# ielym/fastvision

Measured on AMD Instinct MI355X. Metric: images/sec (640×640, bs=32/GPU) YOLOv3 train step, 1/2/4/8 MI355X, higher is better.
Workload: dtype bf16

## Files before the change

fastvision_amd/csrc/conv_wgrad.hip:

```cpp
#include <type_traits>

#include "common.h"

namespace {

__device__ __forceinline__ void wait_vm0() { asm volatile("s_waitcnt vmcnt(0)" ::: "memory"); }
template <int N>
__device__ __forceinline__ void wait_vmcnt_n() {
    asm volatile("s_waitcnt vmcnt(%0)" ::"n"(N) : "memory");
}

__device__ __forceinline__ void slab_store(float* p, float v) { *p = v; }

struct WgradParams {
    const void* x;
    const void* dy;
    float* slab;
    int M, N, C;
    int OW, OHW;
    FastDiv div_ow, div_ohw;
    int x_img, x_row, sy, sx, x_y0, x_x0;
    int dy_img, dy_row, dy_pad, dy_pitch;
    uint32_t dy_zero_off;
    int ntaps;
// ... 298 lines not shown
    __builtin_amdgcn_sched_barrier(0);

    const int i16 = lane & 15, g = lane >> 4, q = i16 >> 2, pp = i16 & 3;
    const uint32_t lds0 = (uint32_t)(size_t)LDS_PTR(smem);
    uint32_t ra[2][4], rb[2][2];
#pragma unroll
    for (int hh = 0; hh < 2; ++hh) {
        const int row = 8 * g + 4 * hh + q;
        const int fr = (q << 2) | ((2 * g + hh) & 3);
        const int rbase = row * 256 + 8 * (pp & 1);
#pragma unroll
        for (int t = 0; t < 4; ++t) ra[hh][t] = lds0 + rbase + (((wr * 8 + t * 2 + (pp >> 1)) ^ fr) << 4);
#pragma unroll
        for (int t = 0; t < 2; ++t) rb[hh][t] = lds0 + rbase + (((wc * 4 + t * 2 + (pp >> 1)) ^ fr) << 4);
    }
    bf16x8 af[4][2], b0[2][2], b1[2][2];
    auto read_a = [&](uint32_t boff, auto kind_tag) {
        constexpr int KO = decltype(kind_tag)::value * OP;
#pragma unroll
        for (int mt = 0; mt < 4; ++mt) {
            af[mt][0] = cat8(tr_read<KO>(ra[0][mt] + boff), tr_read<KO>(ra[1][mt] + boff));
            af[mt][1] = cat8(tr_read<KO + 8192>(ra[0][mt] + boff), tr_read<KO + 8192>(ra[1][mt] + boff));
        }
    };
    auto read_b = [&](uint32_t boff, auto kind_tag, bf16x8 (&bf)[2][2]) {
        constexpr int KO = decltype(kind_tag)::value * OP;
#pragma unroll
        for (int nt = 0; nt < 2; ++nt) {
            bf[nt][0] = cat8(tr_read<KO>(rb[0][nt] + boff), tr_read<KO>(rb[1][nt] + boff));
            bf[nt][1] = cat8(tr_read<KO + 8192>(rb[0][nt] + boff), tr_read<KO + 8192>(rb[1][nt] + boff));
        }
    };
    auto mma = [&](int ha, int hb, bf16x8 (&bf)[2][2]) {
        __builtin_amdgcn_s_setprio(1);
#pragma unroll
        for (int kk = 0; kk < 2; ++kk)
#pragma unroll
            for (int mt = 0; mt < 4; ++mt)
#pragma unroll
                for (int nt = 0; nt < 2; ++nt)
                    acc[ha * 4 + mt][hb * 2 + nt] =
                        __builtin_amdgcn_mfma_f32_16x16x32_bf16(af[mt][kk], bf[nt][kk], acc[ha * 4 + mt][hb * 2 + nt], 0, 0, 0);
        __builtin_amdgcn_s_setprio(0);
    };
    auto retire_reads_then_barrier = [&]() {
        asm volatile("s_waitcnt lgkmcnt(0)" ::: "memory");
        __builtin_amdgcn_s_barrier();
        __builtin_amdgcn_sched_barrier(0);
    };
    using K0 = std::integral_constant<int, 0>;
    using K1 = std::integral_constant<int, 1>;
    using K2 = std::integral_constant<int, 2>;
    using K3 = std::integral_constant<int, 3>;

    uint32_t d1[2], x1[2], d2[2], x2[2];
    {
        uint32_t d0[2], x0[2];
        decode(0, d0, x0);
        stage(2, 0, d0, x0); stage(0, 0, d0, x0); stage(3, 0, d0, x0); stage(1, 0, d0, x0);
    }
    decode(1, d1, x1);
    decode(2, d2, x2);
    if (steps > 1) {
        stage(2, 1, d1, x1); stage(0, 1, d1, x1); stage(3, 1, d1, x1);
        wait_vmcnt_n<6>();
    } else {
        wait_vmcnt_n<0>();
    }
    __builtin_amdgcn_s_barrier();
    stamp(1);
    if (wr == 1) __builtin_amdgcn_s_barrier();

    for (int s = 0; s < steps; ++s) {
        const int cur = s & 1;
        const uint32_t boff = (uint32_t)cur * BUF;
        read_b(boff, K2{}, b0);
        read_a(boff, K0{});
        if (s + 1 < steps) stage(1, cur ^ 1, d1, x1);
        retire_reads_then_barrier();
        mma(0, 0, b0);
        __builtin_amdgcn_s_barrier();
        read_b(boff, K3{}, b1);
        if (s + 2 < steps) stage(2, cur, d2, x2);
        retire_reads_then_barrier();
        mma(0, 1, b1);
        __builtin_amdgcn_s_barrier();
        read_a(boff, K1{});
        if (s + 2 < steps) stage(0, cur, d2, x2);
        retire_reads_then_barrier();
        mma(1, 1, b1);
        __builtin_amdgcn_s_barrier();
        if (s + 2 < steps) {
            stage(3, cur, d2, x2);
            wait_vmcnt_n<6>();
        } else {
            wait_vmcnt_n<0>();
        }
        d1[0] = d2[0]; d1[1] = d2[1]; x1[0] = x2[0]; x1[1] = x2[1];
        decode(s + 3, d2, x2);
        __builtin_amdgcn_s_barrier();
        __builtin_amdgcn_sched_barrier(0);
        mma(1, 0, b0);
        __builtin_amdgcn_s_barrier();
    }
    if (wr == 0) __builtin_amdgcn_s_barrier();
    stamp(2);

    float* out = p.slab + (int64_t)ks * p.ntaps * p.N * p.C;
    const int r = lane & 15;
#pragma unroll
    for (int mi = 0; mi < 8; ++mi)
#pragma unroll
        for (int ni = 0; ni < 4; ++ni) {
            const int j = wc * 64 + ni * 16 + r;
            int tap, c;
            if (p.tpt > 1) {
                const int ts = j / p.C;
                tap = tg * p.tpt + ts;
                c = j - ts * p.C;
            } else {
                tap = tg;
                c = c0 + j;
            }
            if (c < p.C && tap < p.ntaps) {
#pragma unroll
                for (int jj = 0; jj < 4; ++jj) {
                    const int n = n0 + wr * 128 + mi * 16 + g * 4 + jj;
                    if (n < p.N) slab_store(out + ((int64_t)tap * p.N + n) * p.C + c, acc[mi][ni][jj]);
                }
            }
        }
    stamp(3);
}

struct PwgradParams {
    const void* x;
    const void* dy;
    float* slab;
    int B, OH, OW;
    int x_img, x_row, x_y0, x_x0;
    int dy_img, dy_row, dy_pad;
    int tx, ty, tiles, per_block;
    int runs;
    FastDiv div_tx, div_img;
};

template <int V>
struct IntC {
    static constexpr int value = V;
};
template <int I, int N, class F>
__device__ __forceinline__ void static_for(F&& f) {
    if constexpr (I < N) {
        f(IntC<I>{});
        static_for<I + 1, N>(f);
    }
}

template <int C, int NTOT, int STRIDE, int TH>
__global__ __launch_bounds__(256, (C == 32 && TH * STRIDE <= 4) ? 3 : 2) void pwgrad_kernel(const PwgradParams p) {
    constexpr int TW = 32, NB = 64, NH = NTOT / NB;
    constexpr int XW = STRIDE * TW + 2, XH = STRIDE * (TH - 1) + 3, XPIX = XW * XH;
    constexpr int XROWB = C * 2, YROWB = NB * 2;
    constexpr int XPPI = 1024 / XROWB, YPPI = 1024 / YROWB;
    constexpr int X_INSTR = (XPIX + XPPI - 1) / XPPI, Y_INSTR = TH * TW / YPPI;
    constexpr int X_BYTES = X_INSTR * 1024;
    constexpr int WC = C / 16, WN = 4 / WC;
    constexpr int NT = NB / 16 / WN, CT = 9;
    static_assert(9 * (C / 16) == WC * CT && WN * WC == 4, "nine column tiles per wave");
    static_assert((TH - 1) * STRIDE * XW * XROWB + 4 * XROWB < 65536 && (TH - 1) * 32 * YROWB + 4 * YROWB < 65536, "ds_read immediates");
    extern __shared__ __attribute__((aligned(16))) char smem[];
    char* const xs = smem;
    char* const ys = smem + X_BYTES;
    const int tid = threadIdx.x, lane = tid & 63, w = tid >> 6;
    const int wn = w / WC, wc = w % WC;
    const int i16 = lane & 15, g = lane >> 4, q = i16 >> 2, pp = i16 & 3;

    int run, nh;
    if (NH == 1) {
        run = blockIdx.x;
        nh = 0;
    } else {
        const int t = blockIdx.x >> 3;
        nh = t & 1;
        run = (t >> 1) * 8 + (blockIdx.x & 7);
        if (run >= p.runs) return;
    }

    auto xswz = [](int lcol) { return C == 32 ? (lcol >> 3) & 1 : ((lcol >> 1) & 1) | (((lcol >> 3) & 1) << 1); };
    auto yswz = [](int row) { return ((row >> 1) & 1) | (((row >> 3) & 1) << 1); };
    const uint32_t lds_x = (uint32_t)(size_t)LDS_PTR(xs), lds_y = (uint32_t)(size_t)LDS_PTR(ys);

    uint32_t ya[NT], xa[CT][2];
#pragma unroll
    for (int nt = 0; nt < NT; ++nt) {
        const int row0 = 8 * g + q;
        ya[nt] = lds_y + row0 * YROWB + (((wn * NT + nt) ^ yswz(row0)) << 5) + pp * 8;
    }
#pragma unroll
    for (int ct = 0; ct < CT; ++ct) {
        const int gct = wc * CT + ct;
        const int tap = gct / (C / 16), blk = gct % (C / 16);
        const int tyy = tap / 3, txx = tap - 3 * tyy;
        const int off = STRIDE == 1 ? txx : (txx & 1) * (XW / 2) + (txx >> 1);
#pragma unroll
        for (int h = 0; h < 2; ++h) {
            const int lcol = off + 8 * g + q + 4 * h;
            xa[ct][h] = lds_x + (tyy * XW + lcol) * XROWB + ((blk ^ xswz(lcol)) << 5) + pp * 8;
        }
    }

    f32x4 acc[NT][CT];
#pragma unroll
    for (int i = 0; i < NT; ++i)
#pragma unroll
        for (int j = 0; j < CT; ++j) acc[i][j] = f32x4{0.f, 0.f, 0.f, 0.f};

    const int t_begin = run * p.per_block;
    const int t_end = t_begin + p.per_block < p.tiles ? t_begin + p.per_block : p.tiles;
    const int Hx = p.x_img / p.x_row;
#pragma unroll 1
    for (int tile = t_begin; tile < t_end; ++tile) {
        const int b = (int)fd_div((uint32_t)tile, p.div_img);
        const int trem = tile - b * (p.tx * p.ty);
        const int tyi = (int)fd_div((uint32_t)trem, p.div_tx), txi = trem - tyi * p.tx;
        const int oy0 = tyi * TH, ox0 = txi * TW;
        __syncthreads();
        {
        {
            const bf16_t* src0 = (const bf16_t*)p.x + (int64_t)b * p.x_img * C;
#pragma unroll 1
            for (int i = 0; i < (X_INSTR + 3) / 4; ++i) {
                const int j = i * 4 + w;
                if (j < X_INSTR) {
                    const int row = j * XPPI + lane / (XROWB / 16);
                    const int pix = row < XPIX ? row : XPIX - 1;
                    const int py = STRIDE == 1 ? (pix * 1928) >> 16 : (pix * 993) >> 16;
                    const int lcol = pix - py * XW;
                    const int px = STRIDE == 1 ? lcol : (lcol < XW / 2 ? 2 * lcol : 2 * (lcol - XW / 2) + 1);
                    int iy = STRIDE * oy0 + p.x_y0 + py, ix = STRIDE * ox0 + p.x_x0 + px;
                    iy = iy < Hx ? iy : Hx - 1;
                    ix = ix < p.x_row ? ix : p.x_row - 1;
                    const int chunk = (lane % (XROWB / 16)) ^ (xswz(lcol) << 1);
                    __builtin_amdgcn_global_load_lds(GLB_PTR(src0 + ((int64_t)iy * p.x_row + ix) * C + chunk * 8), LDS_PTR(xs + j * 1024), 16, 0, 0);
                }
            }
        }
        {
            const bf16_t* src0 = (const bf16_t*)p.dy + (int64_t)b * p.dy_img * NTOT + nh * NB;
#pragma unroll 1
            for (int i = 0; i < (Y_INSTR + 3) / 4; ++i) {
                const int j = i * 4 + w;
                if (j < Y_INSTR) {
                    const int row = j * YPPI + lane / (YROWB / 16);
                    const int oy = oy0 + (row >> 5), ox = ox0 + (row & 31);
                    const bool in = oy < p.OH && ox < p.OW;
                    const int64_t pix = in ? (int64_t)(oy + p.dy_pad) * p.dy_row + ox + p.dy_pad : 0;
                    const int chunk = (lane % (YROWB / 16)) ^ (yswz(row) << 1);
                    __builtin_amdgcn_global_load_lds(GLB_PTR(src0 + pix * NTOT + chunk * 8), LDS_PTR(ys + j * 1024), 16, 0, 0);
                }
            }
        }
        }
        wait_vm0();
        __syncthreads();
        static_for<0, TH>([&](auto rc) {
            constexpr int r = decltype(rc)::value;
            constexpr int XO = r * STRIDE * XW * XROWB, YO = r * 32 * YROWB;
            constexpr int CG = C == 32 ? 9 : 5;
            bf16x8 af[NT];
#pragma unroll
            for (int nt = 0; nt < NT; ++nt) af[nt] = cat8(tr_read<YO>(ya[nt]), tr_read<YO + 4 * YROWB>(ya[nt]));
#pragma unroll
            for (int c0 = 0; c0 < CT; c0 += CG) {
                bf16x8 bfr[CG];
#pragma unroll
                for (int ct = c0; ct < (c0 + CG < CT ? c0 + CG : CT); ++ct) bfr[ct - c0] = cat8(tr_read<XO>(xa[ct][0]), tr_read<XO>(xa[ct][1]));
                asm volatile("s_waitcnt lgkmcnt(0)" ::: "memory");
                __builtin_amdgcn_sched_barrier(0);
#pragma unroll
                for (int nt = 0; nt < NT; ++nt)
#pragma unroll
                    for (int ct = c0; ct < (c0 + CG < CT ? c0 + CG : CT); ++ct)
                        acc[nt][ct] = __builtin_amdgcn_mfma_f32_16x16x32_bf16(af[nt], bfr[ct - c0], acc[nt][ct], 0, 0, 0);
                __builtin_amdgcn_sched_barrier(0);
            }
        });
    }
    float* out = p.slab + (int64_t)run * 9 * NTOT * C;
#pragma unroll
    for (int nt = 0; nt < NT; ++nt)
#pragma unroll
        for (int ct = 0; ct < CT; ++ct) {
            const int gct = wc * CT + ct;
            const int tap = gct / (C / 16), c = (gct % (C / 16)) * 16 + i16;
#pragma unroll
            for (int j = 0; j < 4; ++j) {
                const int n = nh * NB + (wn * NT + nt) * 16 + g * 4 + j;
                slab_store(out + ((int64_t)tap * NTOT + n) * C + c, acc[nt][ct][j]);
            }
        }
}

__global__ __launch_bounds__(256) void wgrad_reduce_kernel(const float* __restrict__ slab, float* __restrict__ dw, int N, int C,
                                                           int ntaps, int ksplit, int accumulate) {
    __shared__ float part[4][9][64];
    __shared__ float outs[64 * 9];
    const int64_t nc = (int64_t)N * C;
    const int64_t i0 = (int64_t)blockIdx.x * 64;
    const int li = threadIdx.x & 63, grp = threadIdx.x >> 6;
    const int64_t i = i0 + li;
    for (int t = 0; t < ntaps; ++t) {
        float s = 0.f;
        if (i < nc) {
            const float* src = slab + (int64_t)t * nc + i;
            int k = grp;
            for (; k + 12 < ksplit; k += 16) {
                const float v0 = src[(int64_t)k * ntaps * nc], v1 = src[(int64_t)(k + 4) * ntaps * nc];
                const float v2 = src[(int64_t)(k + 8) * ntaps * nc], v3 = src[(int64_t)(k + 12) * ntaps * nc];
                s += (v0 + v1) + (v2 + v3);
            }
            for (; k < ksplit; k += 4) s += src[(int64_t)k * ntaps * nc];
        }
        part[grp][t][li] = s;
    }
    __syncthreads();
    for (int e = threadIdx.x; e < 64 * ntaps; e += 256) {
        const int t = e / 64, l = e - t * 64;
        outs[l * ntaps + t] = (part[0][t][l] + part[1][t][l]) + (part[2][t][l] + part[3][t][l]);
    }
    __syncthreads();
    const int64_t valid = (nc - i0 < 64 ? nc - i0 : 64) * ntaps;
    for (int e = threadIdx.x; e < valid; e += 256) {
        float* o = dw + i0 * ntaps + e;
        *o = accumulate ? *o + outs[e] : outs[e];
    }
}

template <int TAPS>
__global__ __launch_bounds__(1024) void wgrad_reduce4_kernel(const float* __restrict__ slab, float* __restrict__ dw, int N, int C,
                                                             int ksplit, int accumulate, int kg) {
    extern __shared__ float rsm[];
    float* part = rsm;
    float* outs = rsm + kg * TAPS * 256;
    const int64_t nc = (int64_t)N * C;
    const int64_t i0 = (int64_t)blockIdx.x * 256;
    const int li = threadIdx.x & 63, grp = threadIdx.x >> 6;
    const int64_t i = i0 + li * 4;
    const int64_t kstride = (int64_t)TAPS * nc;
    f32x4 s[TAPS];
#pragma unroll
    for (int t = 0; t < TAPS; ++t) s[t] = f32x4{0.f, 0.f, 0.f, 0.f};
    if (i < nc) {
        const float* src = slab + i;
        constexpr int KU = TAPS == 1 ? 8 : 4;
        int k = grp;
        for (; k + (KU - 1) * kg < ksplit; k += KU * kg) {
            f32x4 v[KU][TAPS];
#pragma unroll
            for (int u = 0; u < KU; ++u)
#pragma unroll
                for (int t = 0; t < TAPS; ++t) v[u][t] = *(const f32x4*)(src + (int64_t)(k + u * kg) * kstride + (int64_t)t * nc);
#pragma unroll
            for (int u = 0; u < KU; ++u)
#pragma unroll
                for (int t = 0; t < TAPS; ++t) s[t] += v[u][t];
        }
        for (; k < ksplit; k += kg) {
            f32x4 v[TAPS];
#pragma unroll
            for (int t = 0; t < TAPS; ++t) v[t] = *(const f32x4*)(src + (int64_t)k * kstride + (int64_t)t * nc);
#pragma unroll
            for (int t = 0; t < TAPS; ++t) s[t] += v[t];
        }
    }
#pragma unroll
    for (int t = 0; t < TAPS; ++t) *(f32x4*)(part + ((grp * TAPS + t) * 256 + li * 4)) = s[t];
    __syncthreads();
    for (int e = threadIdx.x; e < 256 * TAPS; e += blockDim.x) {
        const int t = e / 256, l = e - t * 256;
        float a = 0.f;
        for (int g = 0; g < kg; ++g) a += part[(g * TAPS + t) * 256 + l];
        outs[l * TAPS + t] = a;
    }
    __syncthreads();
    const int64_t valid = (nc - i0 < 256 ? nc - i0 : 256) * TAPS;
    for (int e = threadIdx.x; e < valid; e += blockDim.x) {
        float* o = dw + i0 * TAPS + e;
        *o = accumulate ? *o + outs[e] : outs[e];
    }
}

__global__ __launch_bounds__(1024) void wgrad_reduce_tap_kernel(const float* __restrict__ slab, float* __restrict__ dw, int64_t nc, int ksplit,
                                                                int accumulate) {
    __shared__ f32x4 part[16][64];
    const int t = blockIdx.y;
    const int64_t i0 = (int64_t)blockIdx.x * 256;
    const int li = threadIdx.x & 63, w = threadIdx.x >> 6;
    const int64_t i = i0 + li * 4;
    const int64_t kstride = 9 * nc;
    f32x4 s = f32x4{0.f, 0.f, 0.f, 0.f};
    if (i < nc) {
        const float* src = slab + (int64_t)t * nc + i;
        int k = w;
        for (; k + 7 * 16 < ksplit; k += 8 * 16) {
            f32x4 v[8];
#pragma unroll
            for (int u = 0; u < 8; ++u) v[u] = *(const f32x4*)(src + (int64_t)(k + u * 16) * kstride);
#pragma unroll
            for (int u = 0; u < 8; ++u) s += v[u];
        }
        for (; k < ksplit; k += 16) s += *(const f32x4*)(src + (int64_t)k * kstride);
    }
    part[w][li] = s;
    __syncthreads();
    if (threadIdx.x < 256) {
        const int l = threadIdx.x;
        float a = 0.f;
#pragma unroll
        for (int g = 0; g < 16; ++g) a += part[g][l >> 2][l & 3];
        if (i0 + l < nc) {
            float* o = dw + (i0 + l) * 9 + t;
            *o = accumulate ? *o + a : a;
        }
    }
}

struct WgradPlan {
    int tile, ntn, ntc, ntaps, ksplit, mchunk, M, OH, OW, tpt, ngroups;
};

inline bool wgrad_thin_enabled() {
    static bool v = [] {
        const char* e = getenv("FVA_WGRAD_THIN");
        return !e || atoi(e) != 0;
    }();
    return v;
}
inline bool wgrad8_enabled() {
    static bool v = [] {
        const char* e = getenv("FVA_WGRAD8");
        return !e || atoi(e) != 0;
    }();
    return v;
}
inline bool use_wgrad8(const fva_conv_desc* d) {
    if (!wgrad8_enabled() || d->dtype != FVA_BF16 || d->ksize != 3 || d->Cout % 256 || !(d->Cin == 128 || d->Cin % 256 == 0)) return false;
    const int64_t OH = (d->H - 1) / d->stride + 1, OW = (d->W - 1) / d->stride + 1, M = d->B * OH * OW;
    const int64_t units = (int64_t)(d->Cout / 256) * cdiv(d->Cin, 256) * (d->Cin == 128 ? 5 : 9);
    return M * units >= 24ll * 64 * 256;
}

int g_wgrad_plan_beside = 0;
int plan_wgrad(const fva_conv_desc* d, WgradPlan& pl, bool beside = false) {
    pl.tile = d->dtype == FVA_BF16 ? (use_wgrad8(d) ? 256 : 128) : 64;
    pl.OH = (d->H - 1) / d->stride + 1;
    pl.OW = (d->W - 1) / d->stride + 1;
    pl.M = d->B * pl.OH * pl.OW;
    pl.ntn = cdiv(d->Cout, pl.tile);
    pl.ntc = cdiv(d->Cin, pl.tile);
    pl.ntaps = d->ksize * d->ksize;
    pl.tpt = (d->Cin < pl.tile && pl.tile % d->Cin == 0 && pl.ntaps > 1) ? pl.tile / d->Cin : 1;
    pl.ngroups = cdiv(pl.ntaps, pl.tpt);
    const int tiles = pl.ntn * pl.ntc * pl.ngroups;
    const int max_by_m = cdiv(pl.M, 256) > 0 ? cdiv(pl.M, 256) : 1;
    const int64_t per = (int64_t)pl.ntaps * d->Cout * d->Cin * 4;
    int64_t max_by_ws = (512ll << 20) / per;
    int kmax = max_by_m < 1024 ? max_by_m : 1024;
    if (kmax > max_by_ws) kmax = (int)max_by_ws;
    if (kmax < 1) kmax = 1;
    static const int slots8 = [] { const char* e = getenv("FVA_WGRAD_SLOTS8"); return e && atoi(e) > 0 ? atoi(e) : 0; }();
    static const int slots4 = [] { const char* e = getenv("FVA_WGRAD_SLOTS"); return e && atoi(e) > 0 ? atoi(e) : 0; }();
    const int slots = pl.tile == 256 ? (slots8 ? slots8 : beside ? 128 : 256) : (slots4 ? slots4 : beside ? 256 : 512);
    const double t_full = 2.0 * pl.M * pl.tile * pl.tile / (pl.tile == 256 ? 4.3e12 : 1.6e12);
    const double t_slab = (double)per * 2.0 / 3.0e12 + 0.05e-6;
    int ks = 1;
    double best = 1e30;
    for (int k = 1; k <= kmax; ++k) {
        const int rounds = cdiv((int64_t)tiles * k, slots);
        const double cost = rounds * t_full / k + k * t_slab;
        if (cost < best * (1.0 - 1e-9)) { best = cost; ks = k; }
    }
    pl.mchunk = cdiv(cdiv(pl.M, ks), 64) * 64;
    pl.ksplit = cdiv(pl.M, pl.mchunk);
    return FVA_OK;
}

inline bool use_pwgrad(const fva_conv_desc* d) {
    static const bool on = [] { const char* e = getenv("FVA_PWGRAD"); return !e || atoi(e) != 0; }();
    if (!on || d->dtype != FVA_BF16 || d->ksize != 3 || !((d->Cin == 32 && d->Cout == 64) || (d->Cin == 64 && d->Cout == 128))) return false;
    const int OW = (d->W - 1) / d->stride + 1, OH = (d->H - 1) / d->stride + 1;
    return OW >= 32 && OH >= 8 && d->in_pad >= 1 && d->dy_pad >= 1;
}
struct PwgradPlan {
    int th, tx, ty, tiles, runs, per_block, grid;
};
inline int pwgrad_th(const fva_conv_desc* d) {
    static int th1 = 0, th2 = 0;
    static const bool init = [] {
        const char* e = getenv("FVA_PWGRAD_TH");
        if (e) {
            int a = 0, b = 0;
            const int n = sscanf(e, "%d,%d", &a, &b);
            if (n >= 1 && (a == 8 || a == 4)) th1 = a;
            if (n >= 2 && (b == 4 || b == 2)) th2 = b;
        }
        return true;
    }();
    (void)init;
    if (d->stride == 1) return th1 ? th1 : 8;
    return th2 ? th2 : (d->Cin == 64 ? 2 : 4);
}
inline void plan_pwgrad(const fva_conv_desc* d, PwgradPlan& pl, bool beside) {
    const int OH = (d->H - 1) / d->stride + 1, OW = (d->W - 1) / d->stride + 1;
    pl.th = pwgrad_th(d);
    pl.tx = cdiv(OW, 32);
    pl.ty = cdiv(OH, pl.th);
    pl.tiles = d->B * pl.tx * pl.ty;
    const int nh = d->Cout / 64;
    static const int per_cu = [] { const char* e = getenv("FVA_PWGRAD_SLOTS"); return e ? atoi(e) : 2; }();
    int slots = 256 * per_cu / nh;
    if (beside) slots /= 2;
    const int runs = pl.tiles < slots ? pl.tiles : slots;
    pl.per_block = cdiv(pl.tiles, runs);
    pl.runs = cdiv(pl.tiles, pl.per_block);
    pl.grid = nh == 1 ? pl.runs : cdiv(pl.runs, 8) * 16;
}

template <int C, int N, int STRIDE, int TH>
int launch_pwgrad(const PwgradParams& p, int grid, hipStream_t s) {
    constexpr int XPIX = (STRIDE * 32 + 2) * (STRIDE * (TH - 1) + 3);
    constexpr int XPPI = 1024 / (C * 2);
    constexpr int smem = ((XPIX + XPPI - 1) / XPPI) * 1024 + (TH * 32 / 8) * 1024;
    static bool attr_done = false;
    if (!attr_done) {
        (void)hipFuncSetAttribute((const void*)pwgrad_kernel<C, N, STRIDE, TH>, hipFuncAttributeMaxDynamicSharedMemorySize, smem);
        attr_done = true;
    }
    hipLaunchKernelGGL((pwgrad_kernel<C, N, STRIDE, TH>), dim3(grid), dim3(256), smem, s, p);
    FVA_LAUNCH_CHECK("pwgrad_kernel");
    fva_note_kernel("pwgrad");
    return FVA_OK;
}
template <int C, int N>
int launch_pwgrad_any(const PwgradParams& p, int stride, int th, int grid, hipStream_t s) {
    if (stride == 1) return th == 8 ? launch_pwgrad<C, N, 1, 8>(p, grid, s) : launch_pwgrad<C, N, 1, 4>(p, grid, s);
    return th == 4 ? launch_pwgrad<C, N, 2, 4>(p, grid, s) : launch_pwgrad<C, N, 2, 2>(p, grid, s);
}

}

extern "C" {

int64_t fva_conv_wgrad_workspace(const fva_conv_desc* d) {
    if (!d) return 0;
    WgradPlan pl, pb;
    plan_wgrad(d, pl, false);
    plan_wgrad(d, pb, true);
    int ks = pl.ksplit > pb.ksplit ? pl.ksplit : pb.ksplit;
    if (use_pwgrad(d)) {
        PwgradPlan pp;
        plan_pwgrad(d, pp, false);
        ks = ks > pp.runs ? ks : pp.runs;
    }
    return (int64_t)ks * pl.ntaps * d->Cout * d->Cin * 4;
}

int fva_conv_wgrad_plan(int beside) {
    const int prev = g_wgrad_plan_beside;
    if (beside == 0 || beside == 1) g_wgrad_plan_beside = beside;
    return prev;
}

int fva_conv_wgrad(const fva_conv_desc* d, const void* x, const void* dy, float* dw, int accumulate, void* workspace,
                   int64_t workspace_bytes, void* stream) {
    if (!d || !x || !dy || !dw || !workspace) return fva_fail(FVA_ERR_ARG, "fva_conv_wgrad: null pointer");
    if (d->dtype != FVA_F32 && d->dtype != FVA_BF16) return fva_fail(FVA_ERR_ARG, "fva_conv_wgrad: bad dtype");
    if (!((d->ksize == 1 && d->stride == 1) || (d->ksize == 3 && (d->stride == 1 || d->stride == 2))))
        return fva_fail(FVA_ERR_ARG, "fva_conv_wgrad: unsupported ksize/stride");
    const int epc = d->dtype == FVA_BF16 ? 8 : 4;
    if (d->Cin % epc || d->Cout % epc) return fva_fail(FVA_ERR_ARG, "fva_conv_wgrad: channels must be multiples of %d", epc);
    if (d->in_pad < d->ksize / 2) return fva_fail(FVA_ERR_ARG, "fva_conv_wgrad: in_pad too small");
    if (d->dy_pad < 1) return fva_fail(FVA_ERR_ARG, "fva_conv_wgrad: dy buffer needs a zero border (dy_pad >= 1)");
    const int64_t esz = d->dtype == FVA_BF16 ? 2 : 4;
    if ((int64_t)d->B * (d->H + 2 * d->in_pad) * (d->W + 2 * d->in_pad) * d->Cin * esz >= (1ll << 32) ||
        (int64_t)d->B * (d->H + 2) * (d->W + 2) * d->Cout * esz >= (1ll << 32))
        return fva_fail(FVA_ERR_ARG, "fva_conv_wgrad: operand larger than 4 GiB (32-bit byte offsets)");
    WgradPlan pl;
    const bool beside = g_wgrad_plan_beside != 0;
    plan_wgrad(d, pl, beside);
    FvaProfileSpan span(2 | (d->ksize << 8), 2.0 * pl.M * (double)d->Cout * d->Cin * d->ksize * d->ksize, (hipStream_t)stream);
    if (use_pwgrad(d)) {
        PwgradPlan pp;
        plan_pwgrad(d, pp, beside);
        const int64_t need = (int64_t)pp.runs * 9 * d->Cout * d->Cin * 4;
        if (workspace_bytes < need) return fva_fail(FVA_ERR_WORKSPACE, "fva_conv_wgrad: workspace %lld < %lld", (long long)workspace_bytes, (long long)need);
        PwgradParams q = PwgradParams();
        q.x = x; q.dy = dy; q.slab = (float*)workspace;
        q.B = d->B; q.OH = pl.OH; q.OW = pl.OW;
        q.x_row = d->W + 2 * d->in_pad;
        q.x_img = (d->H + 2 * d->in_pad) * q.x_row;
        q.x_y0 = q.x_x0 = d->in_pad - 1;
        q.dy_row = pl.OW + 2 * d->dy_pad;
        q.dy_img = (pl.OH + 2 * d->dy_pad) * q.dy_row;
        q.dy_pad = d->dy_pad;
        q.tx = pp.tx; q.ty = pp.ty; q.tiles = pp.tiles; q.per_block = pp.per_block; q.runs = pp.runs;
        q.div_tx = make_fastdiv(pp.tx);
        q.div_img = make_fastdiv(pp.tx * pp.ty);
        hipStream_t s = (hipStream_t)stream;
        const int rc = d->Cin == 32 ? launch_pwgrad_any<32, 64>(q, d->stride, pp.th, pp.grid, s) : launch_pwgrad_any<64, 128>(q, d->stride, pp.th, pp.grid, s);
        if (rc) return rc;
        const int64_t nc = (int64_t)d->Cout * d->Cin;
        hipLaunchKernelGGL(wgrad_reduce_tap_kernel, dim3((int)((nc + 255) / 256), 9), dim3(1024), 0, s, (const float*)workspace, dw, nc, pp.runs, accumulate);
        FVA_LAUNCH_CHECK("wgrad_reduce_tap_kernel");
        return FVA_OK;
    }
    const int64_t need = (int64_t)pl.ksplit * pl.ntaps * d->Cout * d->Cin * 4;
    if (workspace_bytes < need) return fva_fail(FVA_ERR_WORKSPACE, "fva_conv_wgrad: workspace %lld < %lld", (long long)workspace_bytes, (long long)need);
    WgradParams p = WgradParams();
    p.x = x;
    p.dy = dy;
    p.slab = (float*)workspace;
    p.M = pl.M;
    p.N = d->Cout;
    p.C = d->Cin;
    p.OW = pl.OW;
    p.OHW = pl.OH * pl.OW;
    p.div_ow = make_fastdiv(p.OW);
    p.div_ohw = make_fastdiv(p.OHW);
    p.x_row = d->W + 2 * d->in_pad;
    p.x_img = (d->H + 2 * d->in_pad) * p.x_row;
    p.sy = p.sx = d->stride;
    p.x_y0 = p.x_x0 = d->in_pad - d->ksize / 2;
    p.dy_row = pl.OW + 2 * d->dy_pad;
    p.dy_img = (pl.OH + 2 * d->dy_pad) * p.dy_row;
    p.dy_pad = d->dy_pad;
    p.dy_pitch = d->Cout;
    p.dy_zero_off = 0;
    p.ntaps = pl.ntaps;
    for (int kh = 0; kh < d->ksize; ++kh)
        for (int kw = 0; kw < d->ksize; ++kw) p.tap_pix[kh * d->ksize + kw] = kh * p.x_row + kw;
    p.ntn = pl.ntn;
    p.ntc = pl.ntc;
    p.ksplit = pl.ksplit;
    p.mchunk = pl.mchunk;
    p.tpt = pl.tpt;
    p.ngroups = pl.ngroups;
    const int grid = pl.ksplit * pl.ngroups * pl.ntn * pl.ntc;
    const int smem = 2 * 2 * 64 * 256;
    hipStream_t s = (hipStream_t)stream;
    if (pl.tile == 256) {
        static bool attr_done = false;
        if (!attr_done) {
            (void)hipFuncSetAttribute((const void*)wgrad8_kernel, hipFuncAttributeMaxDynamicSharedMemorySize, 2 * 4 * 64 * 256);
            attr_done = true;
        }
        p.stamps = fva_debug_stamps_ptr();
        p.stamp_rows = fva_debug_stamps_rows();
        hipLaunchKernelGGL(wgrad8_kernel, dim3(grid), dim3(512), 2 * 4 * 64 * 256, s, p);
        fva_note_kernel("wgrad8");
    } else if (d->dtype == FVA_BF16 && d->Cout <= 64 && wgrad_thin_enabled()) {
        hipLaunchKernelGGL((wgrad_kernel<bf16_t, true>), dim3(grid), dim3(256), smem, s, p);
        fva_note_kernel("wgrad128thin");
    } else if (d->dtype == FVA_BF16) {
        hipLaunchKernelGGL(wgrad_kernel<bf16_t>, dim3(grid), dim3(256), smem, s, p);
        fva_note_kernel("wgrad128");
    } else {
        hipLaunchKernelGGL(wgrad_kernel<float>, dim3(grid), dim3(256), smem, s, p);
        fva_note_kernel("wgrad64f32");
    }
    FVA_LAUNCH_CHECK("wgrad_kernel");
    const int64_t nc = (int64_t)d->Cout * d->Cin;
    static const bool reduce4 = [] { const char* e = getenv("FVA_WGRAD_REDUCE4"); return !e || atoi(e) != 0; }();
    if (reduce4 && nc % 4 == 0 && ((uintptr_t)workspace & 15) == 0 && (pl.ntaps == 1 || pl.ntaps == 9)) {
        int kg = 4;
        if (pl.ntaps == 1)
            while (kg < 16 && kg * 8 < pl.ksplit) kg *= 2;
        const int smem_r = (kg + 1) * pl.ntaps * 256 * 4;
        const dim3 grid((int)((nc + 255) / 256)), block(64 * kg);
        if (pl.ntaps == 1) {
            hipLaunchKernelGGL(wgrad_reduce4_kernel<1>, grid, block, smem_r, s, (const float*)workspace, dw, d->Cout, d->Cin, pl.ksplit, accumulate, kg);
        } else {
            static bool attr9 = false;
            if (!attr9) {
                (void)hipFuncSetAttribute((const void*)wgrad_reduce4_kernel<9>, hipFuncAttributeMaxDynamicSharedMemorySize, 5 * 9 * 256 * 4);
                attr9 = true;
            }
            hipLaunchKernelGGL(wgrad_reduce4_kernel<9>, grid, block, smem_r, s, (const float*)workspace, dw, d->Cout, d->Cin, pl.ksplit, accumulate, kg);
        }
    } else
        hipLaunchKernelGGL(wgrad_reduce_kernel, dim3((int)((nc + 63) / 64)), dim3(256), 0, s, (const float*)workspace, dw, d->Cout,
                           d->Cin, pl.ntaps, pl.ksplit, accumulate);
    FVA_LAUNCH_CHECK("wgrad_reduce_kernel");
    return FVA_OK;
}

int fva_stem_wgrad_mfma(const void* img4, const void* dy_halo, float* dw_raw, void* workspace, int64_t workspace_bytes, int B, int H,
                        int W, void* stream) {
    if (!img4 || !dy_halo || !dw_raw || !workspace) return fva_fail(FVA_ERR_ARG, "fva_stem_wgrad_mfma: null pointer");
    const int64_t M = (int64_t)B * H * W;
    if (M >= (1ll << 31) || (int64_t)B * (H + 2) * (W + 2) * 64 >= (1ll << 32)) return fva_fail(FVA_ERR_ARG, "fva_stem_wgrad_mfma: too large");
    const int ksplit_max = 512;
    int mchunk = cdiv(cdiv(M, ksplit_max), 64) * 64;
    const int ksplit = cdiv(M, mchunk);
    const int64_t need = (int64_t)ksplit * 3 * 32 * 16 * 4;
    if (workspace_bytes < need) return fva_fail(FVA_ERR_WORKSPACE, "fva_stem_wgrad_mfma: workspace %lld < %lld", (long long)workspace_bytes, (long long)need);
    WgradParams p = WgradParams();
    p.x = img4;
    p.dy = dy_halo;
    p.slab = (float*)workspace;
    p.M = (int)M;
    p.N = 32;
    p.C = 16;
    p.x_pix_bytes = 8;
    p.OW = W;
    p.OHW = H * W;
    p.div_ow = make_fastdiv(p.OW);
    p.div_ohw = make_fastdiv(p.OHW);
    p.x_row = W + 2;
    p.x_img = (H + 2) * p.x_row;
    p.sy = p.sx = 1;
    p.x_y0 = p.x_x0 = 0;
    p.dy_row = W + 2;
    p.dy_img = (H + 2) * p.dy_row;
    p.dy_pad = 1;
    p.dy_pitch = 32;
    p.dy_zero_off = 0;
    p.ntaps = 3;
    for (int kh = 0; kh < 3; ++kh) p.tap_pix[kh] = kh * p.x_row;
    p.ntn = p.ntc = 1;
    p.ksplit = ksplit;
    p.mchunk = mchunk;
    p.tpt = 8;
    p.ngroups = 1;
    FvaProfileSpan span(2 | (3 << 8), 2.0 * M * 32.0 * 27.0, (hipStream_t)stream);
    hipStream_t s = (hipStream_t)stream;
    if (wgrad_thin_enabled())
        hipLaunchKernelGGL((wgrad_kernel<bf16_t, true>), dim3(ksplit), dim3(256), 2 * 2 * 64 * 256, s, p);
    else
        hipLaunchKernelGGL(wgrad_kernel<bf16_t>, dim3(ksplit), dim3(256), 2 * 2 * 64 * 256, s, p);
    FVA_LAUNCH_CHECK("wgrad_kernel");
    hipLaunchKernelGGL(wgrad_reduce_kernel, dim3((32 * 16 + 63) / 64), dim3(256), 0, s, (const float*)workspace, dw_raw, 32, 16, 3, ksplit, 0);
    FVA_LAUNCH_CHECK("wgrad_reduce_kernel");
    return FVA_OK;
}

int64_t fva_stem_wgrad_mfma_workspace(void) { return 512ll * 3 * 32 * 16 * 4; }

}
```

Measured before the change: 1117.

## Unify wgrad split-K reduce kernels with adaptive tap-split and lane-width grid

Merges the three split-K reduction kernels into one templated kernel with a shared launcher. The launcher picks how many taps each block handles (9, 3 or 1) and, for 1x1 convs, narrows the lane group so small weight tensors still produce enough blocks to fill the GPU. The scalar fallback now splits taps across the grid's y dimension. Env-var knobs for slot counts and the reduce4 path are removed. The aim is better occupancy for small reductions, but it may cost extra launches per tap and less coalesced dw writes when taps are split.

```diff
diff --git a/fastvision_amd/csrc/conv_wgrad.hip b/fastvision_amd/csrc/conv_wgrad.hip
--- a/fastvision_amd/csrc/conv_wgrad.hip
+++ b/fastvision_amd/csrc/conv_wgrad.hip
@@ -624,128 +624,135 @@
         }
 }
 
-__global__ __launch_bounds__(256) void wgrad_reduce_kernel(const float* __restrict__ slab, float* __restrict__ dw, int N, int C,
-                                                           int ntaps, int ksplit, int accumulate) {
-    __shared__ float part[4][9][64];
-    __shared__ float outs[64 * 9];
-    const int64_t nc = (int64_t)N * C;
-    const int64_t i0 = (int64_t)blockIdx.x * 64;
-    const int li = threadIdx.x & 63, grp = threadIdx.x >> 6;
-    const int64_t i = i0 + li;
-    for (int t = 0; t < ntaps; ++t) {
-        float s = 0.f;
-        if (i < nc) {
-            const float* src = slab + (int64_t)t * nc + i;
+template <int V>
+struct ReduceVec {
+    using type = f32x4;
+};
+template <>
+struct ReduceVec<1> {
+    using type = float;
+};
+
+template <int TB, int V>
+__global__ __launch_bounds__(1024) void wgrad_reduce_kernel(const float* __restrict__ slab, float* __restrict__ dw, int64_t nc, int ntaps,
+                                                            int ksplit, int kg, int lg_shift, int accumulate) {
+    static_assert(V == 4 || TB == 1, "the scalar form takes one tap per block");
+    using vec = typename ReduceVec<V>::type;
+    extern __shared__ __attribute__((aligned(16))) float rsm[];
+    const int lg = 1 << lg_shift, ch = lg * V;
+    const int li = threadIdx.x & (lg - 1), grp = threadIdx.x >> lg_shift;
+    const int t0 = blockIdx.y * TB;
+    const int64_t i0 = (int64_t)blockIdx.x * ch;
+    const int64_t i = i0 + li * V;
+    const int64_t kstride = (int64_t)ntaps * nc;
+    vec s[TB];
+#pragma unroll
+    for (int t = 0; t < TB; ++t) s[t] = vec{};
+    if (i < nc) {
+        const float* src = slab + (int64_t)t0 * nc + i;
+        if constexpr (V == 4) {
+            constexpr int KU = TB == 1 ? 8 : 4;
+            int k = grp;
+            for (; k + (KU - 1) * kg < ksplit; k += KU * kg) {
+                vec v[KU][TB];
+#pragma unroll
+                for (int u = 0; u < KU; ++u)
+#pragma unroll
+                    for (int t = 0; t < TB; ++t) v[u][t] = *(const vec*)(src + (int64_t)(k + u * kg) * kstride + (int64_t)t * nc);
+#pragma unroll
+                for (int u = 0; u < KU; ++u)
+#pragma unroll
+                    for (int t = 0; t < TB; ++t) s[t] += v[u][t];
+            }
+            for (; k < ksplit; k += kg) {
+                vec v[TB];
+#pragma unroll
+                for (int t = 0; t < TB; ++t) v[t] = *(const vec*)(src + (int64_t)k * kstride + (int64_t)t * nc);
+#pragma unroll
+                for (int t = 0; t < TB; ++t) s[t] += v[t];
+            }
+        } else {
             int k = grp;
             for (; k + 12 < ksplit; k += 16) {
-                const float v0 = src[(int64_t)k * ntaps * nc], v1 = src[(int64_t)(k + 4) * ntaps * nc];
-                const float v2 = src[(int64_t)(k + 8) * ntaps * nc], v3 = src[(int64_t)(k + 12) * ntaps * nc];
-                s += (v0 + v1) + (v2 + v3);
+                const float v0 = src[(int64_t)k * kstride], v1 = src[(int64_t)(k + 4) * kstride];
+                const float v2 = src[(int64_t)(k + 8) * kstride], v3 = src[(int64_t)(k + 12) * kstride];
+                s[0] += (v0 + v1) + (v2 + v3);
             }
-            for (; k < ksplit; k += 4) s += src[(int64_t)k * ntaps * nc];
-        }
-        part[grp][t][li] = s;
-    }
+            for (; k < ksplit; k += 4) s[0] += src[(int64_t)k * kstride];
+        }
+    }
+#pragma unroll
+    for (int t = 0; t < TB; ++t) *(vec*)(rsm + ((grp * TB + t) * ch + li * V)) = s[t];
     __syncthreads();
-    for (int e = threadIdx.x; e < 64 * ntaps; e += 256) {
-        const int t = e / 64, l = e - t * 64;
-        outs[l * ntaps + t] = (part[0][t][l] + part[1][t][l]) + (part[2][t][l] + part[3][t][l]);
-    }
-    __syncthreads();
-    const int64_t valid = (nc - i0 < 64 ? nc - i0 : 64) * ntaps;
-    for (int e = threadIdx.x; e < valid; e += 256) {
-        float* o = dw + i0 * ntaps + e;
-        *o = accumulate ? *o + outs[e] : outs[e];
-    }
-}
-
-template <int TAPS>
-__global__ __launch_bounds__(1024) void wgrad_reduce4_kernel(const float* __restrict__ slab, float* __restrict__ dw, int N, int C,
-                                                             int ksplit, int accumulate, int kg) {
-    extern __shared__ float rsm[];
-    float* part = rsm;
-    float* outs = rsm + kg * TAPS * 256;
-    const int64_t nc = (int64_t)N * C;
-    const int64_t i0 = (int64_t)blockIdx.x * 256;
-    const int li = threadIdx.x & 63, grp = threadIdx.x >> 6;
-    const int64_t i = i0 + li * 4;
-    const int64_t kstride = (int64_t)TAPS * nc;
-    f32x4 s[TAPS];
-#pragma unroll
-    for (int t = 0; t < TAPS; ++t) s[t] = f32x4{0.f, 0.f, 0.f, 0.f};
-    if (i < nc) {
-        const float* src = slab + i;
-        constexpr int KU = TAPS == 1 ? 8 : 4;
-        int k = grp;
-        for (; k + (KU - 1) * kg < ksplit; k += KU * kg) {
-            f32x4 v[KU][TAPS];
-#pragma unroll
-            for (int u = 0; u < KU; ++u)
-#pragma unroll
-                for (int t = 0; t < TAPS; ++t) v[u][t] = *(const f32x4*)(src + (int64_t)(k + u * kg) * kstride + (int64_t)t * nc);
-#pragma unroll
-            for (int u = 0; u < KU; ++u)
-#pragma unroll
-                for (int t = 0; t < TAPS; ++t) s[t] += v[u][t];
-        }
-        for (; k < ksplit; k += kg) {
-            f32x4 v[TAPS];
-#pragma unroll
-            for (int t = 0; t < TAPS; ++t) v[t] = *(const f32x4*)(src + (int64_t)k * kstride + (int64_t)t * nc);
-#pragma unroll
-            for (int t = 0; t < TAPS; ++t) s[t] += v[t];
-        }
-    }
-#pragma unroll
-    for (int t = 0; t < TAPS; ++t) *(f32x4*)(part + ((grp * TAPS + t) * 256 + li * 4)) = s[t];
-    __syncthreads();
-    for (int e = threadIdx.x; e < 256 * TAPS; e += blockDim.x) {
-        const int t = e / 256, l = e - t * 256;
-        float a = 0.f;
-        for (int g = 0; g < kg; ++g) a += part[(g * TAPS + t) * 256 + l];
-        outs[l * TAPS + t] = a;
-    }
-    __syncthreads();
-    const int64_t valid = (nc - i0 < 256 ? nc - i0 : 256) * TAPS;
-    for (int e = threadIdx.x; e < valid; e += blockDim.x) {
-        float* o = dw + i0 * TAPS + e;
-        *o = accumulate ? *o + outs[e] : outs[e];
-    }
-}
-
-__global__ __launch_bounds__(1024) void wgrad_reduce_tap_kernel(const float* __restrict__ slab, float* __restrict__ dw, int64_t nc, int ksplit,
-                                                                int accumulate) {
-    __shared__ f32x4 part[16][64];
-    const int t = blockIdx.y;
-    const int64_t i0 = (int64_t)blockIdx.x * 256;
-    const int li = threadIdx.x & 63, w = threadIdx.x >> 6;
-    const int64_t i = i0 + li * 4;
-    const int64_t kstride = 9 * nc;
-    f32x4 s = f32x4{0.f, 0.f, 0.f, 0.f};
-    if (i < nc) {
-        const float* src = slab + (int64_t)t * nc + i;
-        int k = w;
-        for (; k + 7 * 16 < ksplit; k += 8 * 16) {
-            f32x4 v[8];
-#pragma unroll
-            for (int u = 0; u < 8; ++u) v[u] = *(const f32x4*)(src + (int64_t)(k + u * 16) * kstride);
-#pragma unroll
-            for (int u = 0; u < 8; ++u) s += v[u];
-        }
-        for (; k < ksplit; k += 16) s += *(const f32x4*)(src + (int64_t)k * kstride);
-    }
-    part[w][li] = s;
-    __syncthreads();
-    if (threadIdx.x < 256) {
-        const int l = threadIdx.x;
-        float a = 0.f;
-#pragma unroll
-        for (int g = 0; g < 16; ++g) a += part[g][l >> 2][l & 3];
-        if (i0 + l < nc) {
-            float* o = dw + (i0 + l) * 9 + t;
+    const int64_t left = nc - i0;
+    const int valid = left < ch ? (int)left : ch;
+    auto combine = [&](int t, int l) {
+        if constexpr (V == 4) {
+            float a = 0.f;
+            for (int g = 0; g < kg; ++g) a += rsm[(g * TB + t) * ch + l];
+            return a;
+        } else {
+            return (rsm[l] + rsm[ch + l]) + (rsm[2 * ch + l] + rsm[3 * ch + l]);
+        }
+    };
+    if constexpr (TB == 1) {
+        for (int l = threadIdx.x; l < valid; l += blockDim.x) {
+            const float a = combine(0, l);
+            float* o = dw + (i0 + l) * ntaps + t0;
             *o = accumulate ? *o + a : a;
         }
-    }
+    } else {
+        float* outs = rsm + kg * TB * ch;
+        for (int e = threadIdx.x; e < ch * TB; e += blockDim.x) {
+            const int t = e / ch, l = e - t * ch;
+            outs[l * TB + t] = combine(t, l);
+        }
+        __syncthreads();
+        for (int e = threadIdx.x; e < valid * TB; e += blockDim.x) {
+            const int l = e / TB, t = e - l * TB;
+            float* o = dw + (i0 + l) * ntaps + t0 + t;
+            *o = accumulate ? *o + outs[e] : outs[e];
+        }
+    }
+}
+
+int launch_wgrad_reduce(const float* slab, float* dw, int64_t nc, int ntaps, int ksplit, int kg, int accumulate, hipStream_t s) {
+    constexpr int kFill = 512;
+    const bool vec = nc % 4 == 0 && ((uintptr_t)slab & 15) == 0 && (ntaps == 1 || ntaps == 9);
+    if (!vec) {
+        hipLaunchKernelGGL((wgrad_reduce_kernel<1, 1>), dim3((unsigned)cdiv(nc, 64), ntaps), dim3(256), 4 * 64 * 4, s, slab, dw, nc, ntaps, ksplit,
+                           4, 6, accumulate);
+        FVA_LAUNCH_CHECK("wgrad_reduce_kernel");
+        return FVA_OK;
+    }
+    int tb = ntaps, lg_shift = 6;
+#if defined(FVA_REDUCE_ALL_TAPS) && FVA_REDUCE_ALL_TAPS
+    while (lg_shift > 4 && cdiv(nc, 4 << lg_shift) < kFill) --lg_shift;
+#else
+    if (ntaps == 9) {
+        const int64_t chunks = cdiv(nc, 256);
+        tb = chunks >= kFill ? 9 : chunks * 3 >= kFill ? 3 : 1;
+    } else {
+        while (lg_shift > 4 && cdiv(nc, 4 << lg_shift) < kFill) --lg_shift;
+    }
+#endif
+    const int ch = 4 << lg_shift;
+    const dim3 grid((unsigned)cdiv(nc, ch), ntaps / tb), block(kg << lg_shift);
+    const int smem = (kg + (tb > 1 ? 1 : 0)) * tb * ch * 4;
+    if (tb == 1) {
+        hipLaunchKernelGGL((wgrad_reduce_kernel<1, 4>), grid, block, smem, s, slab, dw, nc, ntaps, ksplit, kg, lg_shift, accumulate);
+    } else if (tb == 3) {
+        hipLaunchKernelGGL((wgrad_reduce_kernel<3, 4>), grid, block, smem, s, slab, dw, nc, ntaps, ksplit, kg, lg_shift, accumulate);
+    } else {
+        static bool attr9 = false;
+        if (!attr9) {
+            (void)hipFuncSetAttribute((const void*)wgrad_reduce_kernel<9, 4>, hipFuncAttributeMaxDynamicSharedMemorySize, 64 * 1024);
+            attr9 = true;
+        }
+        hipLaunchKernelGGL((wgrad_reduce_kernel<9, 4>), grid, block, smem, s, slab, dw, nc, ntaps, ksplit, kg, lg_shift, accumulate);
+    }
+    FVA_LAUNCH_CHECK("wgrad_reduce_kernel");
+    return FVA_OK;
 }
 
 struct WgradPlan {
@@ -791,9 +798,7 @@
     int kmax = max_by_m < 1024 ? max_by_m : 1024;
     if (kmax > max_by_ws) kmax = (int)max_by_ws;
     if (kmax < 1) kmax = 1;
-    static const int slots8 = [] { const char* e = getenv("FVA_WGRAD_SLOTS8"); return e && atoi(e) > 0 ? atoi(e) : 0; }();
-    static const int slots4 = [] { const char* e = getenv("FVA_WGRAD_SLOTS"); return e && atoi(e) > 0 ? atoi(e) : 0; }();
-    const int slots = pl.tile == 256 ? (slots8 ? slots8 : beside ? 128 : 256) : (slots4 ? slots4 : beside ? 256 : 512);
+    const int slots = pl.tile == 256 ? (beside ? 128 : 256) : (beside ? 256 : 512);
     const double t_full = 2.0 * pl.M * pl.tile * pl.tile / (pl.tile == 256 ? 4.3e12 : 1.6e12);
     const double t_slab = (double)per * 2.0 / 3.0e12 + 0.05e-6;
     int ks = 1;
@@ -932,10 +937,7 @@
         hipStream_t s = (hipStream_t)stream;
         const int rc = d->Cin == 32 ? launch_pwgrad_any<32, 64>(q, d->stride, pp.th, pp.grid, s) : launch_pwgrad_any<64, 128>(q, d->stride, pp.th, pp.grid, s);
         if (rc) return rc;
-        const int64_t nc = (int64_t)d->Cout * d->Cin;
-        hipLaunchKernelGGL(wgrad_reduce_tap_kernel, dim3((int)((nc + 255) / 256), 9), dim3(1024), 0, s, (const float*)workspace, dw, nc, pp.runs, accumulate);
-        FVA_LAUNCH_CHECK("wgrad_reduce_tap_kernel");
-        return FVA_OK;
+        return launch_wgrad_reduce((const float*)workspace, dw, (int64_t)d->Cout * d->Cin, 9, pp.runs, 16, accumulate, s);
     }
     const int64_t need = (int64_t)pl.ksplit * pl.ntaps * d->Cout * d->Cin * 4;
     if (workspace_bytes < need) return fva_fail(FVA_ERR_WORKSPACE, "fva_conv_wgrad: workspace %lld < %lld", (long long)workspace_bytes, (long long)need);
@@ -993,28 +995,10 @@
     }
     FVA_LAUNCH_CHECK("wgrad_kernel");
     const int64_t nc = (int64_t)d->Cout * d->Cin;
-    static const bool reduce4 = [] { const char* e = getenv("FVA_WGRAD_REDUCE4"); return !e || atoi(e) != 0; }();
-    if (reduce4 && nc % 4 == 0 && ((uintptr_t)workspace & 15) == 0 && (pl.ntaps == 1 || pl.ntaps == 9)) {
-        int kg = 4;
-        if (pl.ntaps == 1)
-            while (kg < 16 && kg * 8 < pl.ksplit) kg *= 2;
-        const int smem_r = (kg + 1) * pl.ntaps * 256 * 4;
-        const dim3 grid((int)((nc + 255) / 256)), block(64 * kg);
-        if (pl.ntaps == 1) {
-            hipLaunchKernelGGL(wgrad_reduce4_kernel<1>, grid, block, smem_r, s, (const float*)workspace, dw, d->Cout, d->Cin, pl.ksplit, accumulate, kg);
-        } else {
-            static bool attr9 = false;
-            if (!attr9) {
-                (void)hipFuncSetAttribute((const void*)wgrad_reduce4_kernel<9>, hipFuncAttributeMaxDynamicSharedMemorySize, 5 * 9 * 256 * 4);
-                attr9 = true;
-            }
-            hipLaunchKernelGGL(wgrad_reduce4_kernel<9>, grid, block, smem_r, s, (const float*)workspace, dw, d->Cout, d->Cin, pl.ksplit, accumulate, kg);
-        }
-    } else
-        hipLaunchKernelGGL(wgrad_reduce_kernel, dim3((int)((nc + 63) / 64)), dim3(256), 0, s, (const float*)workspace, dw, d->Cout,
-                           d->Cin, pl.ntaps, pl.ksplit, accumulate);
-    FVA_LAUNCH_CHECK("wgrad_reduce_kernel");
-    return FVA_OK;
+    int kg = 4;
+    if (pl.ntaps == 1)
+        while (kg < 16 && kg * 8 < pl.ksplit) kg *= 2;
+    return launch_wgrad_reduce((const float*)workspace, dw, nc, pl.ntaps, pl.ksplit, kg, accumulate, s);
 }
 
 int fva_stem_wgrad_mfma(const void* img4, const void* dy_halo, float* dw_raw, void* workspace, int64_t workspace_bytes, int B, int H,
@@ -1062,9 +1046,7 @@
     else
         hipLaunchKernelGGL(wgrad_kernel<bf16_t>, dim3(ksplit), dim3(256), 2 * 2 * 64 * 256, s, p);
     FVA_LAUNCH_CHECK("wgrad_kernel");
-    hipLaunchKernelGGL(wgrad_reduce_kernel, dim3((32 * 16 + 63) / 64), dim3(256), 0, s, (const float*)workspace, dw_raw, 32, 16, 3, ksplit, 0);
-    FVA_LAUNCH_CHECK("wgrad_reduce_kernel");
-    return FVA_OK;
+    return launch_wgrad_reduce((const float*)workspace, dw_raw, 32 * 16, 3, ksplit, 4, 0, s);
 }
 
 int64_t fva_stem_wgrad_mfma_workspace(void) { return 512ll * 3 * 32 * 16 * 4; }
```

After: 1114. No clear change (-0.3%).
